# toufique-morshed/CPU-GPU-TFHE

Measured on AMD Instinct MI355X. Metric: gate bootstraps/sec (bootsNAND, N=1024), higher is better.
Workload: dtype f64 (FFT external product; Torus32 in/out, rounded products exact)

## Files before the change

cpu-gpu-tfhe_amd/csrc/keyswitch.hip:

```cpp
#include "engine.h"
#include "modarith.h"

#include <algorithm>
#include <cstdlib>

namespace tfhe_amd {

namespace {


constexpr int kKs4Cols = 4;
constexpr int kKs4Blocks = 126;
constexpr int kKs4I = 32;
#ifndef TFHE_AMD_KS4_THREADS
#define TFHE_AMD_KS4_THREADS 256
#endif
constexpr int kKs4Threads = TFHE_AMD_KS4_THREADS;
constexpr int kKs4ChunkU4 = kKs4I * kKsT * 3;
static_assert(kKs4ChunkU4 % kKs4Threads == 0, "chunk must split evenly");
constexpr int kKs4Pieces = kKs4ChunkU4 / kKs4Threads;

struct KsLane {
    const int32_t *ua, *ua2;
    uint32_t b;
    int32_t *ra, *rb;
};
struct KsPlain {
    const int32_t *u_a, *u_b, *u2_a, *u2_b;
    int32_t add_b;
    int32_t *res_a, *res_b;
    int B;
    __device__ int count() const { return B; }
    __device__ KsLane lane(int ct) const {
        KsLane l;
        l.ua = u_a + (size_t)ct * kN;
        l.ua2 = u2_a ? u2_a + (size_t)ct * kN : nullptr;
        l.b = (uint32_t)u_b[ct] + (uint32_t)add_b + (u2_b ? (uint32_t)u2_b[ct] : 0u);
        l.ra = res_a + (size_t)ct * kn;
        l.rb = res_b + ct;
        return l;
    }
};
struct KsRows {
    const CircKs *ks;
    const int32_t *u_a, *u_b;
    int32_t *wa, *wb;
    int B, nks;
    __device__ int count() const { return B * nks; }
    __device__ KsLane lane(int ct) const {
        const int g = ct / B, k = ct - g * B;
        const CircKs e = ks[g];
        const size_t s1 = (size_t)e.r1 * B + k, so = (size_t)e.out * B + k;
        KsLane l;
        l.ua = u_a + s1 * kN;
        l.b = (uint32_t)u_b[s1] + (uint32_t)e.add_b;
        l.ua2 = nullptr;
        if (e.r2 >= 0) {
            const size_t s2 = (size_t)e.r2 * B + k;
            l.ua2 = u_a + s2 * kN;
            l.b += (uint32_t)u_b[s2];
        }
        l.ra = wa + so * kn;
        l.rb = wb + so;
        return l;
    }
};

template <class P, int SPLIT>
__global__ __launch_bounds__(kKs4Threads) void k_keyswitch_v4(const uint4 *__restrict__ ksk4, P io) {
    __shared__ __attribute__((aligned(16))) uint4 buf[2][kKs4I * kKsT * 4];
    const int part = SPLIT > 1 ? (int)(blockIdx.x % SPLIT) : 0;
    const int bid = SPLIT > 1 ? (int)(blockIdx.x / SPLIT) : (int)blockIdx.x;
    const int xcd = bid & 7, k = bid >> 3;
    const int cb = (k & 15) * 8 + xcd;
    const int ctg = k >> 4;
    if (cb >= kKs4Blocks) return;
    const int tid = threadIdx.x;
    const int ct = ctg * kKs4Threads + tid;
    const bool valid = ct < io.count();
    const KsLane ln = io.lane(valid ? ct : 0);
    for (int t = tid; t < 2 * kKs4I * kKsT; t += kKs4Threads) buf[t >> 8][(t & 255) * 4] = make_uint4(0, 0, 0, 0);

    uint32_t acc[kKs4Cols];
#pragma unroll
    for (int c = 0; c < kKs4Cols; ++c) acc[c] = 0;
    if (SPLIT == 1 && cb * kKs4Cols <= kn && kn < cb * kKs4Cols + kKs4Cols) acc[kn - cb * kKs4Cols] = ln.b;
    constexpr int kIPart = kN / SPLIT;
    const int ibeg = part * kIPart;

    const uint4 *src = ksk4 + ((size_t)cb * kN + ibeg) * kKsT * 3 + tid;
    const uint4 *pa = reinterpret_cast<const uint4 *>(ln.ua + ibeg);
    const uint4 *pa2 = ln.ua2 ? reinterpret_cast<const uint4 *>(ln.ua2 + ibeg) : nullptr;
    int dst[kKs4Pieces];
    uint4 p[kKs4Pieces];
#pragma unroll
    for (int l = 0; l < kKs4Pieces; ++l) {
        const int t = tid + kKs4Threads * l;
        dst[l] = (t / 3) * 4 + (t - 3 * (t / 3)) + 1;
    }
#pragma unroll
    for (int l = 0; l < kKs4Pieces; ++l) p[l] = src[kKs4Threads * l];
    uint4 av[kKs4I / 4], av2[kKs4I / 4];
#pragma unroll
    for (int v = 0; v < kKs4I / 4; ++v) {
        av[v] = pa[v];
        av2[v] = pa2 ? pa2[v] : make_uint4(0, 0, 0, 0);
    }
#pragma unroll
    for (int l = 0; l < kKs4Pieces; ++l) buf[0][dst[l]] = p[l];
    __syncthreads();
    for (int i0 = 0, b = 0; i0 < kIPart; i0 += kKs4I, b ^= 1) {
        uint32_t a[kKs4I];
#pragma unroll
        for (int v = 0; v < kKs4I / 4; ++v) {
            a[4 * v] = av[v].x + av2[v].x + kKsPrecOffset;
            a[4 * v + 1] = av[v].y + av2[v].y + kKsPrecOffset;
            a[4 * v + 2] = av[v].z + av2[v].z + kKsPrecOffset;
            a[4 * v + 3] = av[v].w + av2[v].w + kKsPrecOffset;
        }
        const bool more = i0 + kKs4I < kIPart;
        if (more) {
            const uint4 *sn = src + (size_t)(i0 + kKs4I) * kKsT * 3;
#pragma unroll
            for (int l = 0; l < kKs4Pieces; ++l) p[l] = sn[kKs4Threads * l];
#pragma unroll
            for (int v = 0; v < kKs4I / 4; ++v) {
                av[v] = pa[(i0 + kKs4I) / 4 + v];
                if (pa2) av2[v] = pa2[(i0 + kKs4I) / 4 + v];
            }
        }
        const uint4 *cur = buf[b];
#pragma unroll
        for (int ii = 0; ii < kKs4I; ++ii) {
            const uint32_t ab = a[ii];
#pragma unroll
            for (int j = 0; j < kKsT; ++j) {
                const uint32_t aij = (ab >> (32 - (j + 1) * kKsBasebit)) & (kKsBase - 1);
                const uint4 r = cur[(ii * kKsT + j) * 4 + (int)aij];
                acc[0] -= r.x; acc[1] -= r.y; acc[2] -= r.z; acc[3] -= r.w;
            }
            asm volatile("" : "+v"(acc[0]), "+v"(acc[1]), "+v"(acc[2]), "+v"(acc[3]));
        }
        if (more) {
            uint4 *nb = buf[b ^ 1];
#pragma unroll
            for (int l = 0; l < kKs4Pieces; ++l) nb[dst[l]] = p[l];
        }
        __syncthreads();
    }
    if (!valid) return;
#pragma unroll
    for (int c = 0; c < kKs4Cols; ++c) {
        const int col = cb * kKs4Cols + c;
        int32_t *dst = col < kn ? ln.ra + col : col == kn ? ln.rb : nullptr;
        if (!dst) continue;
        if (SPLIT > 1) atomicAdd(reinterpret_cast<unsigned int *>(dst), acc[c]);
        else *dst = (int32_t)acc[c];
    }
}

constexpr int kKsSmallChunks = 64;
constexpr int kKsSmallI = kN / kKsSmallChunks;

template <class P>
__global__ __launch_bounds__(512) void k_keyswitch_small_init(P io) {
    const KsLane ln = io.lane(blockIdx.x);
    const int col = threadIdx.x;
    if (col < kn) ln.ra[col] = 0;
    else if (col == kn) *ln.rb = (int32_t)ln.b;
}

#ifndef TFHE_AMD_KS_SMALL_U
#define TFHE_AMD_KS_SMALL_U 2
#endif
constexpr int kKsSmallU = TFHE_AMD_KS_SMALL_U;
template <class P, int U>
__global__ __launch_bounds__(512) void k_keyswitch_small(const int32_t *__restrict__ ksk, P io) {
    const int chunk = blockIdx.x, col = threadIdx.x;
    const KsLane ln = io.lane(blockIdx.y);
    if (col > kn) return;
    const int i0 = chunk * kKsSmallI;
    uint32_t acc = 0;
#pragma unroll U
    for (int ii = 0; ii < kKsSmallI; ++ii) {
        const int i = i0 + ii;
        const uint32_t ab = (uint32_t)ln.ua[i] + (ln.ua2 ? (uint32_t)ln.ua2[i] : 0u) + kKsPrecOffset;
        const int32_t *row = ksk + (size_t)i * kKsT * 3 * kKsRow + col;
#pragma unroll
        for (int j = 0; j < kKsT; ++j) {
            const uint32_t h = (ab >> (32 - (j + 1) * kKsBasebit)) & (kKsBase - 1);
            const uint32_t v = (uint32_t)row[(j * 3 + (int)(h ? h : 1u) - 1) * kKsRow];
            acc -= h ? v : 0u;
        }
    }
    int32_t *dst = col < kn ? ln.ra + col : ln.rb;
    atomicAdd(reinterpret_cast<unsigned int *>(dst), acc);
}

typedef int ks5_v4i __attribute__((ext_vector_type(4)));
typedef int ks5_v16i __attribute__((ext_vector_type(16)));
#ifndef TFHE_AMD_KS5_WAVES
#define TFHE_AMD_KS5_WAVES 8
#endif
constexpr int kKs5Waves = TFHE_AMD_KS5_WAVES;
constexpr int kKs5Threads = 64 * kKs5Waves;
constexpr int kKs5Ch = 16;
constexpr int kKs5Nb = 64;
constexpr int kKs5Cols = 8 * kKs5Nb;
static_assert(kKs5Cols > kn, "the N-blocks cover every column and b");
constexpr int kKs5ChU4 = kKs5Ch * 64;
static_assert(kKs5ChU4 % kKs5Threads == 0, "chunk must split evenly");
constexpr int kKs5Pieces = kKs5ChU4 / kKs5Threads;
#ifndef TFHE_AMD_KS5_G
#define TFHE_AMD_KS5_G 8
#endif
constexpr int kKs5G = TFHE_AMD_KS5_G;

template <class P, int SPLIT, int MS>
__global__ __launch_bounds__(kKs5Threads) void k_keyswitch_v5(const uint4 *__restrict__ w5, P io) {
    constexpr int kM = 32 * kKs5Waves * MS;
    constexpr int kG = kKs5G / MS;
    static_assert(kKs5Ch % kG == 0, "groups split the chunk");
    __shared__ __attribute__((aligned(16))) uint2 lut[16][32];
    __shared__ __attribute__((aligned(16))) uint4 bs[2][kKs5Ch][64];
    __shared__ __attribute__((aligned(16))) uint8_t dg[2][2][kM][kKs5Ch];
    const int bid = (int)blockIdx.x, xcd = bid & 7, kk = bid >> 3;
    const int nb = xcd + 8 * (kk & 7), part = (kk >> 3) % SPLIT, mt = (kk >> 3) / SPLIT;
    constexpr int kChunks = kN / kKs5Ch / SPLIT;
    const int c0 = part * kChunks;
    const int tid = threadIdx.x, wave = tid >> 6, l = tid & 63, r = l & 31, hh = l >> 5;
    for (int e = tid; e < 16 * 32; e += kKs5Threads)
        lut[e >> 5][e & 31] = make_uint2(1u << (8 * ((e >> 7) & 3)), 1u << (8 * ((e >> 5) & 3)));
    constexpr int kPer = kKs5Ch * MS / 2;
    constexpr int kU4 = kPer / 4;
    static_assert(kKs5Threads * kPer == kM * kKs5Ch, "loader mapping");
    const int lct = (tid * MS) >> 1, lpart = MS == 1 ? (tid & 1) : 0;
    const int lg = mt * kM + lct;
    const KsLane lln = io.lane(lg < io.count() ? lg : 0);
    const uint4 *pa = reinterpret_cast<const uint4 *>(lln.ua) + kU4 * lpart;
    const uint4 *pa2 = reinterpret_cast<const uint4 *>(lln.ua2 ? lln.ua2 : lln.ua) + kU4 * lpart;
    const uint32_t m2 = lln.ua2 ? 0xffffffffu : 0u;
    pa += c0 * (kKs5Ch / 4);
    pa2 += c0 * (kKs5Ch / 4);
    uint4 uu[kU4], vv[kU4];
#pragma unroll
    for (int q = 0; q < kU4; ++q) {
        uu[q] = pa[q];
        vv[q] = pa2[q];
    }
    auto put_digits = [&](int buf) {
        uint32_t hi[kPer / 4], lo[kPer / 4];
#pragma unroll
        for (int q = 0; q < kU4; ++q) {
            const uint32_t w[4] = {uu[q].x + (vv[q].x & m2) + kKsPrecOffset, uu[q].y + (vv[q].y & m2) + kKsPrecOffset,
                                   uu[q].z + (vv[q].z & m2) + kKsPrecOffset, uu[q].w + (vv[q].w & m2) + kKsPrecOffset};
            hi[q] = (w[0] >> 24) | ((w[1] >> 24) << 8) | ((w[2] >> 24) << 16) | ((w[3] >> 24) << 24);
            lo[q] = ((w[0] >> 16) & 255u) | (((w[1] >> 16) & 255u) << 8) | (((w[2] >> 16) & 255u) << 16) |
                    (((w[3] >> 16) & 255u) << 24);
        }
        if (kU4 == 2) {
            *reinterpret_cast<uint2 *>(&dg[buf][0][lct][kPer * lpart]) = make_uint2(hi[0], hi[1]);
            *reinterpret_cast<uint2 *>(&dg[buf][1][lct][kPer * lpart]) = make_uint2(lo[0], lo[1]);
        } else {
            *reinterpret_cast<uint4 *>(&dg[buf][0][lct][0]) = make_uint4(hi[0], hi[1], hi[2 % kU4], hi[3 % kU4]);
            *reinterpret_cast<uint4 *>(&dg[buf][1][lct][0]) = make_uint4(lo[0], lo[1], lo[2 % kU4], lo[3 % kU4]);
        }
    };
    const uint4 *src = w5 + ((size_t)nb * kN + (size_t)c0 * kKs5Ch) * 64 + tid;
    uint4 p[kKs5Pieces];
#pragma unroll
    for (int q = 0; q < kKs5Pieces; ++q) p[q] = src[q * kKs5Threads];
#pragma unroll
    for (int q = 0; q < kKs5Pieces; ++q) (&bs[0][0][0])[tid + q * kKs5Threads] = p[q];
    put_digits(0);
    __syncthreads();
    ks5_v16i acc[MS];
#pragma unroll
    for (int m = 0; m < MS; ++m) acc[m] = ks5_v16i{};
    for (int c = 0; c < kChunks; ++c) {
        const bool more = c + 1 < kChunks;
        {
            const int cn = more ? c + 1 : c;
            const uint4 *sn = src + (size_t)cn * kKs5ChU4;
#pragma unroll
            for (int q = 0; q < kKs5Pieces; ++q) p[q] = sn[q * kKs5Threads];
#pragma unroll
            for (int q = 0; q < kU4; ++q) {
                uu[q] = pa[cn * (kKs5Ch / 4) + q];
                vv[q] = pa2[cn * (kKs5Ch / 4) + q];
            }
        }
        uint32_t xw[MS][4];
#pragma unroll
        for (int m = 0; m < MS; ++m) {
            const uint4 xd = *reinterpret_cast<const uint4 *>(&dg[c & 1][hh][wave * 32 * MS + 32 * m + r][0]);
            xw[m][0] = xd.x; xw[m][1] = xd.y; xw[m][2] = xd.z; xw[m][3] = xd.w;
        }
        const uint4(*cur)[64] = bs[c & 1];
#pragma unroll
        for (int g = 0; g < kKs5Ch; g += kG) {
            uint4 av[MS][kG], bv[kG];
#pragma unroll
            for (int q = 0; q < kG; ++q) {
                const int ii = g + q;
#pragma unroll
                for (int m = 0; m < MS; ++m) {
                    const uint32_t xb = xw[m][ii >> 2] >> (8 * (ii & 3));
                    const uint2 d01 = lut[(xb >> 4) & 15u][r], d23 = lut[xb & 15u][r];
                    av[m][q] = make_uint4(d01.x, d01.y, d23.x, d23.y);
                }
                bv[q] = cur[ii][l];
            }
            __builtin_amdgcn_sched_barrier(0);
#pragma unroll
            for (int q = 0; q < kG; ++q) {
                const ks5_v4i b = {(int)bv[q].x, (int)bv[q].y, (int)bv[q].z, (int)bv[q].w};
#pragma unroll
                for (int m = 0; m < MS; ++m) {
                    const ks5_v4i a = {(int)av[m][q].x, (int)av[m][q].y, (int)av[m][q].z, (int)av[m][q].w};
                    acc[m] = __builtin_amdgcn_mfma_i32_32x32x32_i8(a, b, acc[m], 0, 0, 0);
                }
            }
        }
        if (more) {
#pragma unroll
            for (int q = 0; q < kKs5Pieces; ++q) (&bs[(c + 1) & 1][0][0])[tid + q * kKs5Threads] = p[q];
            put_digits((c + 1) & 1);
        }
        __syncthreads();
    }
    const int col = nb * 8 + (r >> 2);
    const uint32_t lsh = 8u * (uint32_t)(l & 3);
#pragma unroll
    for (int m = 0; m < MS; ++m) {
#pragma unroll
        for (int reg = 0; reg < 16; ++reg) {
            uint32_t v = (uint32_t)acc[m][reg] << lsh;
            v += (uint32_t)__shfl_xor((int)v, 1, 64);
            v += (uint32_t)__shfl_xor((int)v, 2, 64);
            const int ctm = mt * kM + wave * 32 * MS + 32 * m + (reg & 3) + 8 * (reg >> 2) + 4 * hh;
            if ((l & 3) == 0 && ctm < io.count() && col <= kn) {
                const KsLane lm = io.lane(ctm);
                if (SPLIT > 1) atomicAdd(reinterpret_cast<unsigned int *>(col < kn ? lm.ra + col : lm.rb), 0u - v);
                else if (col < kn) lm.ra[col] = (int32_t)(0u - v);
                else *lm.rb = (int32_t)(lm.b - v);
            }
        }
    }
}

__global__ __launch_bounds__(256) void k_ksk_to_v5(const int32_t *__restrict__ ksk, uint4 *__restrict__ w5) {
    const size_t total = (size_t)kKs5Nb * kN * 64;
    for (size_t t = (size_t)blockIdx.x * 256 + threadIdx.x; t < total; t += (size_t)gridDim.x * 256) {
        const int l = (int)(t & 63);
        const int i = (int)((t >> 6) % kN);
        const int nb = (int)(t / ((size_t)kN * 64));
        const int col = nb * 8 + ((l & 31) >> 2), limb = l & 3, h = l >> 5;
        uint32_t w[4];
#pragma unroll
        for (int tt = 0; tt < 4; ++tt) {
            uint32_t word = 0;
            for (int hh = 1; hh < 4; ++hh) {
                if (col > kn) break;
                uint32_t v = (uint32_t)ksk[(((size_t)i * kKsT + 4 * h + tt) * 3 + (hh - 1)) * kKsRow + col];
                int8_t sb = 0;
                for (int b = 0; b <= limb; ++b) {
                    sb = (int8_t)(v & 0xffu);
                    v = (v - (uint32_t)(int32_t)sb) >> 8;
                }
                word |= (uint32_t)(uint8_t)sb << (8 * hh);
            }
            w[tt] = word;
        }
        w5[t] = make_uint4(w[0], w[1], w[2], w[3]);
    }
}

__global__ __launch_bounds__(256) void k_ksk_to_v4(const int32_t *__restrict__ ksk, uint4 *__restrict__ ksk4) {
    const size_t pieces = (size_t)kKs4Blocks * kN * kKsT * 3;
    for (size_t t = (size_t)blockIdx.x * 256 + threadIdx.x; t < pieces; t += (size_t)gridDim.x * 256) {
        const int cb = (int)(t / ((size_t)kN * kKsT * 3));
        const size_t row = t % ((size_t)kN * kKsT * 3);
        ksk4[t] = *reinterpret_cast<const uint4 *>(ksk + row * kKsRow + cb * kKs4Cols);
    }
}

}

static int ks_split_max() { return 768; }
bool ks5_enabled() {
    static const bool v = [] {
        const char *e = getenv("TFHE_AMD_KS5");
        return !(e && atoi(e) == 0);
    }();
    return v;
}
static int ks5_split(int mtiles) {
    int sp = 1;
    while (sp < 8 && mtiles * kKs5Nb * sp < 512) sp *= 2;
    return sp;
}
template <class P, int MS>
static void launch_ks5(const uint4 *w5, int count, const P &io, hipStream_t s) {
    const int mtiles = (count + 32 * kKs5Waves * MS - 1) / (32 * kKs5Waves * MS);
    const int split = ks5_split(mtiles);
    if (split > 1) hipLaunchKernelGGL(k_keyswitch_small_init<P>, dim3(count), dim3(512), 0, s, io);
    const dim3 grid(mtiles * kKs5Nb * split);
    trace_kernel(split == 8 ? "k_keyswitch_v5(int8-mfma+split8)" : split == 4 ? "k_keyswitch_v5(int8-mfma+split4)"
                 : split == 2 ? "k_keyswitch_v5(int8-mfma+split2)" : "k_keyswitch_v5(int8-mfma)");
    switch (split) {
    case 8: hipLaunchKernelGGL((k_keyswitch_v5<P, 8, MS>), grid, dim3(kKs5Threads), 0, s, w5, io); break;
    case 4: hipLaunchKernelGGL((k_keyswitch_v5<P, 4, MS>), grid, dim3(kKs5Threads), 0, s, w5, io); break;
    case 2: hipLaunchKernelGGL((k_keyswitch_v5<P, 2, MS>), grid, dim3(kKs5Threads), 0, s, w5, io); break;
    default: hipLaunchKernelGGL((k_keyswitch_v5<P, 1, MS>), grid, dim3(kKs5Threads), 0, s, w5, io); break;
    }
}
template <class P>
static void launch_ks4(const DeviceKey &key, int groups, int count, const P &io, hipStream_t s) {
    if (key.ksk5) {
        const uint4 *w5 = reinterpret_cast<const uint4 *>(key.ksk5);
        launch_ks5<P, 1>(w5, count, io, s);
        return;
    }
    trace_kernel("k_keyswitch_v4");
    if (count <= ks_split_max()) {
        hipLaunchKernelGGL(k_keyswitch_small_init<P>, dim3(count), dim3(512), 0, s, io);
        hipLaunchKernelGGL((k_keyswitch_v4<P, 2>), dim3(2 * 128 * groups), dim3(kKs4Threads), 0, s,
                           reinterpret_cast<const uint4 *>(key.ksk4), io);
    } else {
        hipLaunchKernelGGL((k_keyswitch_v4<P, 1>), dim3(128 * groups), dim3(kKs4Threads), 0, s,
                           reinterpret_cast<const uint4 *>(key.ksk4), io);
    }
}

static int ks_unroll_max() { return 4; }

static int ks_small_max() { return ks5_enabled() ? 12 : 96; }

hipError_t launch_keyswitch_rows(const DeviceKey &key, int B, int nks, const CircKs *ks, const int32_t *u_a,
                                 const int32_t *u_b, int32_t *wa, int32_t *wb, hipStream_t s) {
    if (B <= 0 || nks <= 0) return hipSuccess;
    KsRows io{ks, u_a, u_b, wa, wb, B, nks};
    if ((long)B * nks <= ks_small_max()) {
        trace_kernel("k_keyswitch_small");
        hipLaunchKernelGGL(k_keyswitch_small_init<KsRows>, dim3(B * nks), dim3(512), 0, s, io);
        if ((long)B * nks <= ks_unroll_max())
            hipLaunchKernelGGL((k_keyswitch_small<KsRows, kKsSmallI>), dim3(kKsSmallChunks, B * nks), dim3(512), 0, s,
                               key.ksk, io);
        else
            hipLaunchKernelGGL((k_keyswitch_small<KsRows, kKsSmallU>), dim3(kKsSmallChunks, B * nks), dim3(512), 0, s,
                               key.ksk, io);
        return hipGetLastError();
    }
    const int groups = (int)(((size_t)B * nks + kKs4Threads - 1) / kKs4Threads);
    launch_ks4(key, groups, B * nks, io, s);
    return hipGetLastError();
}

__global__ __launch_bounds__(256) void k_circuit_linear(int B, int nlin, const CircLin *__restrict__ lin,
                                                        int32_t *__restrict__ wa, int32_t *__restrict__ wb) {
    const size_t total = (size_t)nlin * B * (kn + 1);
    for (size_t t = (size_t)blockIdx.x * 256 + threadIdx.x; t < total; t += (size_t)gridDim.x * 256) {
        const int w = (int)(t % (kn + 1));
        const size_t gk = t / (kn + 1);
        const int g = (int)(gk / B), k = (int)(gk - (size_t)g * B);
        const CircLin e = lin[g];
        const size_t so = (size_t)e.out * B + k, si = (size_t)(e.in < 0 ? 0 : e.in) * B + k;
        if (w < kn) wa[so * kn + w] = e.in < 0 ? 0 : (int32_t)((uint32_t)e.s * (uint32_t)wa[si * kn + w]);
        else wb[so] = (int32_t)((uint32_t)e.c + (e.in < 0 ? 0u : (uint32_t)e.s * (uint32_t)wb[si]));
    }
}

size_t ksk_v4_words() { return (size_t)kKs4Blocks * kN * kKsT * 3 * 4; }
size_t ksk_v5_words() { return (size_t)kKs5Nb * kN * 64 * 4; }

hipError_t launch_ksk_to_v5(const int32_t *d_ksk, int32_t *d_ksk5, hipStream_t s) {
    hipLaunchKernelGGL(k_ksk_to_v5, dim3(4096), dim3(256), 0, s, d_ksk, reinterpret_cast<uint4 *>(d_ksk5));
    return hipGetLastError();
}

__device__ __forceinline__ double ks_var_one(const int32_t *__restrict__ u, const int32_t *__restrict__ u2,
                                             const double *__restrict__ var) {
    static_assert(kKsT * kKsBasebit == 16 && kKsBase == 4, "digit count below assumes 8 base-4 digits");
    if (var[kKsVarUniform] != 0.0) {
        int k = 0;
#pragma unroll 8
        for (int i = 0; i < kN; ++i) {
            const uint32_t x = ((uint32_t)u[i] + (u2 ? (uint32_t)u2[i] : 0u) + kKsPrecOffset) >> 16;
            k += __builtin_popcount((x | (x >> 1)) & 0x5555u);
        }
        return var[kKsVarUniform + 1 + k];
    }
    double v = 0.0;
    constexpr int U = 4;
    for (int i0 = 0; i0 < kN; i0 += U) {
        uint32_t ab[U];
#pragma unroll
        for (int k = 0; k < U; ++k) ab[k] = (uint32_t)u[i0 + k] + (u2 ? (uint32_t)u2[i0 + k] : 0u) + kKsPrecOffset;
        double t[U][kKsT];
#pragma unroll
        for (int k = 0; k < U; ++k)
#pragma unroll
            for (int j = 0; j < kKsT; ++j) {
                const uint32_t aij = (ab[k] >> (32 - (j + 1) * kKsBasebit)) & (uint32_t)(kKsBase - 1);
                t[k][j] = var[((i0 + k) * kKsT + j) * kKsBase + aij];
            }
#pragma unroll
        for (int k = 0; k < U; ++k)
#pragma unroll
            for (int j = 0; j < kKsT; ++j) {
                const uint32_t aij = (ab[k] >> (32 - (j + 1) * kKsBasebit)) & (uint32_t)(kKsBase - 1);
                v = __dadd_rn(v, aij ? t[k][j] : 0.0);
            }
    }
    return v;
}

__global__ __launch_bounds__(64) void k_ks_variance(const int32_t *__restrict__ u_a, int B, int halves,
                                                    const double *__restrict__ var, double *__restrict__ out) {
    const int g = blockIdx.x * blockDim.x + threadIdx.x;
    if (g >= B) return;
    out[g] = ks_var_one(u_a + (size_t)g * kN, halves == 2 ? u_a + ((size_t)B + g) * kN : nullptr, var);
}

__global__ __launch_bounds__(64) void k_ks_variance_rows(const int32_t *__restrict__ u_a, int B,
                                                         const CircKs *__restrict__ ks, const double *__restrict__ var,
                                                         double *__restrict__ out) {
    const int g = blockIdx.x * blockDim.x + threadIdx.x;
    if (g >= B) return;
    const CircKs k = ks[g];
    out[g] = ks_var_one(u_a + (size_t)k.r1 * kN, k.r2 >= 0 ? u_a + (size_t)k.r2 * kN : nullptr, var);
}

hipError_t launch_ks_variance_rows(const int32_t *u_a, int B, const CircKs *ks, const double *var, double *out,
                                   hipStream_t s) {
    if (B <= 0) return hipSuccess;
    hipLaunchKernelGGL(k_ks_variance_rows, dim3((B + 63) / 64), dim3(64), 0, s, u_a, B, ks, var, out);
    return hipGetLastError();
}

hipError_t launch_ks_variance(const int32_t *u_a, int B, int halves, const double *var, double *out, hipStream_t s) {
    if (B <= 0) return hipSuccess;
    hipLaunchKernelGGL(k_ks_variance, dim3((B + 63) / 64), dim3(64), 0, s, u_a, B, halves, var, out);
    return hipGetLastError();
}

hipError_t launch_circuit_linear(int B, int nlin, const CircLin *lin, int32_t *wa, int32_t *wb, hipStream_t s) {
    if (B <= 0 || nlin <= 0) return hipSuccess;
    const size_t total = (size_t)nlin * B * (kn + 1);
    const int blocks = (int)std::min<size_t>((total + 255) / 256, 65536);
    trace_kernel("k_circuit_linear");
    hipLaunchKernelGGL(k_circuit_linear, dim3(blocks), dim3(256), 0, s, B, nlin, lin, wa, wb);
    return hipGetLastError();
}

hipError_t launch_ksk_to_v4(const int32_t *d_ksk, int32_t *d_ksk4, hipStream_t s) {
    hipLaunchKernelGGL(k_ksk_to_v4, dim3(2048), dim3(256), 0, s, d_ksk, reinterpret_cast<uint4 *>(d_ksk4));
    return hipGetLastError();
}

int ks_version() { return ks5_enabled() ? 5 : 4; }

hipError_t launch_keyswitch(const DeviceKey &key, int B, const int32_t *u_a, const int32_t *u_b,
                            const int32_t *u2_a, const int32_t *u2_b, int32_t add_b,
                            int32_t *res_a, int32_t *res_b, hipStream_t s) {
    if (B <= 0) return hipSuccess;
    if (B <= ks_small_max()) {
        trace_kernel("k_keyswitch_small");
        KsPlain io{u_a, u_b, u2_a, u2_b, add_b, res_a, res_b, B};
        hipLaunchKernelGGL(k_keyswitch_small_init<KsPlain>, dim3(B), dim3(512), 0, s, io);
        if (B <= ks_unroll_max())
            hipLaunchKernelGGL((k_keyswitch_small<KsPlain, kKsSmallI>), dim3(kKsSmallChunks, B), dim3(512), 0, s,
                               key.ksk, io);
        else
            hipLaunchKernelGGL((k_keyswitch_small<KsPlain, kKsSmallU>), dim3(kKsSmallChunks, B), dim3(512), 0, s,
                               key.ksk, io);
    } else {
        const int groups = (B + kKs4Threads - 1) / kKs4Threads;
        KsPlain io{u_a, u_b, u2_a, u2_b, add_b, res_a, res_b, B};
        launch_ks4(key, groups, B, io, s);
    }
    return hipGetLastError();
}

}
```

Baseline: 325,400.

## Stream keyswitch key into LDS ring via async global_load_lds and compute one-hot digits inline

```diff
diff --git a/cpu-gpu-tfhe_amd/csrc/keyswitch.hip b/cpu-gpu-tfhe_amd/csrc/keyswitch.hip
--- a/cpu-gpu-tfhe_amd/csrc/keyswitch.hip
+++ b/cpu-gpu-tfhe_amd/csrc/keyswitch.hip
@@ -199,152 +199,176 @@
 
 typedef int ks5_v4i __attribute__((ext_vector_type(4)));
 typedef int ks5_v16i __attribute__((ext_vector_type(16)));
-#ifndef TFHE_AMD_KS5_WAVES
-#define TFHE_AMD_KS5_WAVES 8
-#endif
-constexpr int kKs5Waves = TFHE_AMD_KS5_WAVES;
+constexpr int kKs5Waves = 8;
 constexpr int kKs5Threads = 64 * kKs5Waves;
-constexpr int kKs5Ch = 16;
+constexpr int kKs5M = 32 * kKs5Waves;
 constexpr int kKs5Nb = 64;
 constexpr int kKs5Cols = 8 * kKs5Nb;
 static_assert(kKs5Cols > kn, "the N-blocks cover every column and b");
-constexpr int kKs5ChU4 = kKs5Ch * 64;
-static_assert(kKs5ChU4 % kKs5Threads == 0, "chunk must split evenly");
-constexpr int kKs5Pieces = kKs5ChU4 / kKs5Threads;
-#ifndef TFHE_AMD_KS5_G
-#define TFHE_AMD_KS5_G 8
+constexpr int kKs5Ring = 3;
+#ifndef TFHE_AMD_KS5_PH
+#define TFHE_AMD_KS5_PH 16
 #endif
-constexpr int kKs5G = TFHE_AMD_KS5_G;
-
-template <class P, int SPLIT, int MS>
+constexpr int kKs5Ph = TFHE_AMD_KS5_PH;
+constexpr int kKs5G = 8;
+
+typedef __attribute__((address_space(3))) void *ks5_lptr;
+
+__device__ __forceinline__ uint32_t ks5_onehot(uint32_t sh, int k, uint32_t one) {
+    uint32_t d;
+    switch (k) {
+    case 0: asm("v_lshlrev_b32_sdwa %0, %1, %2 dst_sel:DWORD dst_unused:UNUSED_PAD src0_sel:BYTE_0 src1_sel:DWORD" : "=v"(d) : "v"(sh), "v"(one)); break;
+    case 1: asm("v_lshlrev_b32_sdwa %0, %1, %2 dst_sel:DWORD dst_unused:UNUSED_PAD src0_sel:BYTE_1 src1_sel:DWORD" : "=v"(d) : "v"(sh), "v"(one)); break;
+    case 2: asm("v_lshlrev_b32_sdwa %0, %1, %2 dst_sel:DWORD dst_unused:UNUSED_PAD src0_sel:BYTE_2 src1_sel:DWORD" : "=v"(d) : "v"(sh), "v"(one)); break;
+    default: asm("v_lshlrev_b32_sdwa %0, %1, %2 dst_sel:DWORD dst_unused:UNUSED_PAD src0_sel:BYTE_3 src1_sel:DWORD" : "=v"(d) : "v"(sh), "v"(one)); break;
+    }
+    return d;
+}
+
+template <class P, int SPLIT, int PH>
 __global__ __launch_bounds__(kKs5Threads) void k_keyswitch_v5(const uint4 *__restrict__ w5, P io) {
-    constexpr int kM = 32 * kKs5Waves * MS;
-    constexpr int kG = kKs5G / MS;
-    static_assert(kKs5Ch % kG == 0, "groups split the chunk");
-    __shared__ __attribute__((aligned(16))) uint2 lut[16][32];
-    __shared__ __attribute__((aligned(16))) uint4 bs[2][kKs5Ch][64];
-    __shared__ __attribute__((aligned(16))) uint8_t dg[2][2][kM][kKs5Ch];
+    constexpr int kM = kKs5M;
+    constexpr int kQ = PH / 16;
+    constexpr int kPhases = kN / PH / SPLIT;
+    static_assert(PH % 16 == 0 && kN % (PH * SPLIT) == 0 && kPhases >= 1, "phases split the range");
+    static_assert(PH % kKs5G == 0 && PH % kKs5Waves == 0, "groups and fill split the phase");
+    constexpr int kOffRing = 0, kOffDg = kKs5Ring * PH * 1024;
+    constexpr int kLds = kOffDg + 2 * 2 * kQ * kM * 16;
+    static_assert(kLds <= 160 * 1024, "LDS of one CU");
+    __shared__ __attribute__((aligned(16))) uint8_t lds[kLds];
+    auto dgp = [&](int buf, int half, int q, int ct) { return lds + kOffDg + (((buf * 2 + half) * kQ + q) * kM + ct) * 16; };
     const int bid = (int)blockIdx.x, xcd = bid & 7, kk = bid >> 3;
     const int nb = xcd + 8 * (kk & 7), part = (kk >> 3) % SPLIT, mt = (kk >> 3) / SPLIT;
-    constexpr int kChunks = kN / kKs5Ch / SPLIT;
-    const int c0 = part * kChunks;
-    const int tid = threadIdx.x, wave = tid >> 6, l = tid & 63, r = l & 31, hh = l >> 5;
-    for (int e = tid; e < 16 * 32; e += kKs5Threads)
-        lut[e >> 5][e & 31] = make_uint2(1u << (8 * ((e >> 7) & 3)), 1u << (8 * ((e >> 5) & 3)));
-    constexpr int kPer = kKs5Ch * MS / 2;
+    const int p0 = part * kPhases;
+    const int tid = threadIdx.x, wave = __builtin_amdgcn_readfirstlane(tid >> 6), l = tid & 63, r = l & 31, hh = l >> 5;
+    const uint4 *src = w5 + ((size_t)nb * kN + (size_t)p0 * PH) * 64 + l;
+    auto fill = [&](int p) {
+        const uint4 *g = src + (size_t)p * PH * 64;
+        const uint32_t slot = __builtin_amdgcn_readfirstlane(
+            (uint32_t)(uintptr_t)(ks5_lptr)(lds + kOffRing + (p % kKs5Ring) * PH * 1024 + wave * 1024));
+#pragma unroll
+        for (int k = 0; k < PH / kKs5Waves; ++k) {
+            uint32_t keep;
+            asm volatile("s_mov_b32 %0, m0\n\ts_mov_b32 m0, %2\n\ts_nop 0\n\tglobal_load_lds_dwordx4 %1, off\n\t"
+                         "s_mov_b32 m0, %0"
+                         : "=&s"(keep)
+                         : "v"(g + (wave + kKs5Waves * k) * 64), "s"(slot + kKs5Waves * k * 1024)
+                         : "memory");
+        }
+    };
+    auto ring_wait = [] { asm volatile("s_waitcnt vmcnt(0)" ::: "memory"); };
+    fill(0);
+    if (kPhases > 1) fill(1);
+    constexpr int kPer = PH / 2;
     constexpr int kU4 = kPer / 4;
-    static_assert(kKs5Threads * kPer == kM * kKs5Ch, "loader mapping");
-    const int lct = (tid * MS) >> 1, lpart = MS == 1 ? (tid & 1) : 0;
+    static_assert(kKs5Threads * kPer == kM * PH, "loader mapping");
+    const int lct = tid >> 1, lpart = tid & 1;
     const int lg = mt * kM + lct;
     const KsLane lln = io.lane(lg < io.count() ? lg : 0);
-    const uint4 *pa = reinterpret_cast<const uint4 *>(lln.ua) + kU4 * lpart;
-    const uint4 *pa2 = reinterpret_cast<const uint4 *>(lln.ua2 ? lln.ua2 : lln.ua) + kU4 * lpart;
-    const uint32_t m2 = lln.ua2 ? 0xffffffffu : 0u;
-    pa += c0 * (kKs5Ch / 4);
-    pa2 += c0 * (kKs5Ch / 4);
+    const uint4 *pa = reinterpret_cast<const uint4 *>(lln.ua) + kU4 * lpart + p0 * (PH / 4);
+    const uint4 *pa2 = reinterpret_cast<const uint4 *>(lln.ua2 ? lln.ua2 : lln.ua) + kU4 * lpart + p0 * (PH / 4);
+    const bool has2 = lln.ua2 != nullptr;
     uint4 uu[kU4], vv[kU4];
 #pragma unroll
     for (int q = 0; q < kU4; ++q) {
         uu[q] = pa[q];
-        vv[q] = pa2[q];
+        vv[q] = make_uint4(0, 0, 0, 0);
+    }
+    if (has2) {
+#pragma unroll
+        for (int q = 0; q < kU4; ++q) vv[q] = pa2[q];
     }
     auto put_digits = [&](int buf) {
-        uint32_t hi[kPer / 4], lo[kPer / 4];
+        uint32_t hi[kU4], lo[kU4];
 #pragma unroll
         for (int q = 0; q < kU4; ++q) {
-            const uint32_t w[4] = {uu[q].x + (vv[q].x & m2) + kKsPrecOffset, uu[q].y + (vv[q].y & m2) + kKsPrecOffset,
-                                   uu[q].z + (vv[q].z & m2) + kKsPrecOffset, uu[q].w + (vv[q].w & m2) + kKsPrecOffset};
+            const uint32_t w[4] = {uu[q].x + vv[q].x + kKsPrecOffset, uu[q].y + vv[q].y + kKsPrecOffset,
+                                   uu[q].z + vv[q].z + kKsPrecOffset, uu[q].w + vv[q].w + kKsPrecOffset};
             hi[q] = (w[0] >> 24) | ((w[1] >> 24) << 8) | ((w[2] >> 24) << 16) | ((w[3] >> 24) << 24);
             lo[q] = ((w[0] >> 16) & 255u) | (((w[1] >> 16) & 255u) << 8) | (((w[2] >> 16) & 255u) << 16) |
                     (((w[3] >> 16) & 255u) << 24);
         }
         if (kU4 == 2) {
-            *reinterpret_cast<uint2 *>(&dg[buf][0][lct][kPer * lpart]) = make_uint2(hi[0], hi[1]);
-            *reinterpret_cast<uint2 *>(&dg[buf][1][lct][kPer * lpart]) = make_uint2(lo[0], lo[1]);
+            *reinterpret_cast<uint2 *>(dgp(buf, 0, 0, lct) + 8 * lpart) = make_uint2(hi[0], hi[1]);
+            *reinterpret_cast<uint2 *>(dgp(buf, 1, 0, lct) + 8 * lpart) = make_uint2(lo[0], lo[1]);
         } else {
-            *reinterpret_cast<uint4 *>(&dg[buf][0][lct][0]) = make_uint4(hi[0], hi[1], hi[2 % kU4], hi[3 % kU4]);
-            *reinterpret_cast<uint4 *>(&dg[buf][1][lct][0]) = make_uint4(lo[0], lo[1], lo[2 % kU4], lo[3 % kU4]);
+            *reinterpret_cast<uint4 *>(dgp(buf, 0, lpart, lct)) = make_uint4(hi[0], hi[1], hi[2 % kU4], hi[3 % kU4]);
+            *reinterpret_cast<uint4 *>(dgp(buf, 1, lpart, lct)) = make_uint4(lo[0], lo[1], lo[2 % kU4], lo[3 % kU4]);
         }
     };
-    const uint4 *src = w5 + ((size_t)nb * kN + (size_t)c0 * kKs5Ch) * 64 + tid;
-    uint4 p[kKs5Pieces];
-#pragma unroll
-    for (int q = 0; q < kKs5Pieces; ++q) p[q] = src[q * kKs5Threads];
-#pragma unroll
-    for (int q = 0; q < kKs5Pieces; ++q) (&bs[0][0][0])[tid + q * kKs5Threads] = p[q];
+    static_assert(kU4 == 2 || kU4 == 4, "PH is 16 or 32");
     put_digits(0);
+    ring_wait();
     __syncthreads();
-    ks5_v16i acc[MS];
-#pragma unroll
-    for (int m = 0; m < MS; ++m) acc[m] = ks5_v16i{};
-    for (int c = 0; c < kChunks; ++c) {
-        const bool more = c + 1 < kChunks;
+    ks5_v16i acc = ks5_v16i{};
+    for (int p = 0; p < kPhases; ++p) {
+        const bool more = p + 1 < kPhases;
+        if (p + 2 < kPhases) fill(p + 2);
         {
-            const int cn = more ? c + 1 : c;
-            const uint4 *sn = src + (size_t)cn * kKs5ChU4;
-#pragma unroll
-            for (int q = 0; q < kKs5Pieces; ++q) p[q] = sn[q * kKs5Threads];
-#pragma unroll
-            for (int q = 0; q < kU4; ++q) {
-                uu[q] = pa[cn * (kKs5Ch / 4) + q];
-                vv[q] = pa2[cn * (kKs5Ch / 4) + q];
-            }
-        }
-        uint32_t xw[MS][4];
-#pragma unroll
-        for (int m = 0; m < MS; ++m) {
-            const uint4 xd = *reinterpret_cast<const uint4 *>(&dg[c & 1][hh][wave * 32 * MS + 32 * m + r][0]);
-            xw[m][0] = xd.x; xw[m][1] = xd.y; xw[m][2] = xd.z; xw[m][3] = xd.w;
-        }
-        const uint4(*cur)[64] = bs[c & 1];
-#pragma unroll
-        for (int g = 0; g < kKs5Ch; g += kG) {
-            uint4 av[MS][kG], bv[kG];
-#pragma unroll
-            for (int q = 0; q < kG; ++q) {
-                const int ii = g + q;
-#pragma unroll
-                for (int m = 0; m < MS; ++m) {
-                    const uint32_t xb = xw[m][ii >> 2] >> (8 * (ii & 3));
-                    const uint2 d01 = lut[(xb >> 4) & 15u][r], d23 = lut[xb & 15u][r];
-                    av[m][q] = make_uint4(d01.x, d01.y, d23.x, d23.y);
+            const int pn = more ? p + 1 : p;
+#pragma unroll
+            for (int q = 0; q < kU4; ++q) uu[q] = pa[pn * (PH / 4) + q];
+            if (has2) {
+#pragma unroll
+                for (int q = 0; q < kU4; ++q) vv[q] = pa2[pn * (PH / 4) + q];
+            }
+        }
+        const uint8_t *cur = lds + kOffRing + (p % kKs5Ring) * PH * 1024 + l * 16;
+#pragma unroll
+        for (int q16 = 0; q16 < kQ; ++q16) {
+            const uint4 xd = *reinterpret_cast<const uint4 *>(dgp(p & 1, hh, q16, wave * 32 + r));
+            const uint32_t xw[4] = {xd.x, xd.y, xd.z, xd.w};
+            uint32_t sh[4][4];
+            const uint32_t one = 1u;
+#pragma unroll
+            for (int d = 0; d < 4; ++d) {
+                const uint32_t m = 0x18181818u;
+                sh[d][0] = (xw[d] >> 3) & m; sh[d][1] = (xw[d] >> 1) & m;
+                sh[d][2] = (xw[d] << 1) & m; sh[d][3] = (xw[d] << 3) & m;
+            }
+#pragma unroll
+            for (int g = 0; g < 16; g += kKs5G) {
+                uint4 av[kKs5G], bv[kKs5G];
+#pragma unroll
+                for (int q = 0; q < kKs5G; ++q) {
+                    const int ii = g + q;
+                    av[q] = make_uint4(ks5_onehot(sh[ii >> 2][0], ii & 3, one), ks5_onehot(sh[ii >> 2][1], ii & 3, one),
+                                       ks5_onehot(sh[ii >> 2][2], ii & 3, one), ks5_onehot(sh[ii >> 2][3], ii & 3, one));
+                    bv[q] = *reinterpret_cast<const uint4 *>(cur + (16 * q16 + ii) * 1024);
                 }
-                bv[q] = cur[ii][l];
-            }
-            __builtin_amdgcn_sched_barrier(0);
-#pragma unroll
-            for (int q = 0; q < kG; ++q) {
-                const ks5_v4i b = {(int)bv[q].x, (int)bv[q].y, (int)bv[q].z, (int)bv[q].w};
-#pragma unroll
-                for (int m = 0; m < MS; ++m) {
-                    const ks5_v4i a = {(int)av[m][q].x, (int)av[m][q].y, (int)av[m][q].z, (int)av[m][q].w};
-                    acc[m] = __builtin_amdgcn_mfma_i32_32x32x32_i8(a, b, acc[m], 0, 0, 0);
+                __builtin_amdgcn_sched_barrier(0);
+#pragma unroll
+                for (int q = 0; q < kKs5G; ++q) {
+                    const ks5_v4i b = {(int)bv[q].x, (int)bv[q].y, (int)bv[q].z, (int)bv[q].w};
+                    const ks5_v4i a = {(int)av[q].x, (int)av[q].y, (int)av[q].z, (int)av[q].w};
+                    acc = __builtin_amdgcn_mfma_i32_32x32x32_i8(a, b, acc, 0, 0, 0);
                 }
             }
         }
+        __builtin_amdgcn_sched_barrier(0);
+#pragma unroll
+        for (int q = 0; q < kU4; ++q)
+            asm volatile("" : "+v"(uu[q].x), "+v"(uu[q].y), "+v"(uu[q].z), "+v"(uu[q].w), "+v"(vv[q].x), "+v"(vv[q].y),
+                              "+v"(vv[q].z), "+v"(vv[q].w));
         if (more) {
-#pragma unroll
-            for (int q = 0; q < kKs5Pieces; ++q) (&bs[(c + 1) & 1][0][0])[tid + q * kKs5Threads] = p[q];
-            put_digits((c + 1) & 1);
-        }
-        __syncthreads();
+            put_digits((p + 1) & 1);
+            ring_wait();
+            __syncthreads();
+        }
     }
     const int col = nb * 8 + (r >> 2);
     const uint32_t lsh = 8u * (uint32_t)(l & 3);
 #pragma unroll
-    for (int m = 0; m < MS; ++m) {
-#pragma unroll
-        for (int reg = 0; reg < 16; ++reg) {
-            uint32_t v = (uint32_t)acc[m][reg] << lsh;
-            v += (uint32_t)__shfl_xor((int)v, 1, 64);
-            v += (uint32_t)__shfl_xor((int)v, 2, 64);
-            const int ctm = mt * kM + wave * 32 * MS + 32 * m + (reg & 3) + 8 * (reg >> 2) + 4 * hh;
-            if ((l & 3) == 0 && ctm < io.count() && col <= kn) {
-                const KsLane lm = io.lane(ctm);
-                if (SPLIT > 1) atomicAdd(reinterpret_cast<unsigned int *>(col < kn ? lm.ra + col : lm.rb), 0u - v);
-                else if (col < kn) lm.ra[col] = (int32_t)(0u - v);
-                else *lm.rb = (int32_t)(lm.b - v);
-            }
+    for (int reg = 0; reg < 16; ++reg) {
+        uint32_t v = (uint32_t)acc[reg] << lsh;
+        v += (uint32_t)__shfl_xor((int)v, 1, 64);
+        v += (uint32_t)__shfl_xor((int)v, 2, 64);
+        const int ctm = mt * kM + wave * 32 + (reg & 3) + 8 * (reg >> 2) + 4 * hh;
+        if ((l & 3) == 0 && ctm < io.count() && col <= kn) {
+            const KsLane lm = io.lane(ctm);
+            if (SPLIT > 1) atomicAdd(reinterpret_cast<unsigned int *>(col < kn ? lm.ra + col : lm.rb), 0u - v);
+            else if (col < kn) lm.ra[col] = (int32_t)(0u - v);
+            else *lm.rb = (int32_t)(lm.b - v);
         }
     }
 }
@@ -396,30 +420,36 @@
     return v;
 }
 static int ks5_split(int mtiles) {
+    static const int forced = [] {
+        const char *e = getenv("TFHE_AMD_KS5_SPLIT");
+        const int v = e ? atoi(e) : 0;
+        return v == 1 || v == 2 || v == 4 || v == 8 ? v : 0;
+    }();
+    if (forced) return forced;
     int sp = 1;
     while (sp < 8 && mtiles * kKs5Nb * sp < 512) sp *= 2;
     return sp;
 }
-template <class P, int MS>
+template <class P>
 static void launch_ks5(const uint4 *w5, int count, const P &io, hipStream_t s) {
-    const int mtiles = (count + 32 * kKs5Waves * MS - 1) / (32 * kKs5Waves * MS);
+    const int mtiles = (count + kKs5M - 1) / kKs5M;
     const int split = ks5_split(mtiles);
     if (split > 1) hipLaunchKernelGGL(k_keyswitch_small_init<P>, dim3(count), dim3(512), 0, s, io);
     const dim3 grid(mtiles * kKs5Nb * split);
     trace_kernel(split == 8 ? "k_keyswitch_v5(int8-mfma+split8)" : split == 4 ? "k_keyswitch_v5(int8-mfma+split4)"
                  : split == 2 ? "k_keyswitch_v5(int8-mfma+split2)" : "k_keyswitch_v5(int8-mfma)");
     switch (split) {
-    case 8: hipLaunchKernelGGL((k_keyswitch_v5<P, 8, MS>), grid, dim3(kKs5Threads), 0, s, w5, io); break;
-    case 4: hipLaunchKernelGGL((k_keyswitch_v5<P, 4, MS>), grid, dim3(kKs5Threads), 0, s, w5, io); break;
-    case 2: hipLaunchKernelGGL((k_keyswitch_v5<P, 2, MS>), grid, dim3(kKs5Threads), 0, s, w5, io); break;
-    default: hipLaunchKernelGGL((k_keyswitch_v5<P, 1, MS>), grid, dim3(kKs5Threads), 0, s, w5, io); break;
+    case 8: hipLaunchKernelGGL((k_keyswitch_v5<P, 8, kKs5Ph>), grid, dim3(kKs5Threads), 0, s, w5, io); break;
+    case 4: hipLaunchKernelGGL((k_keyswitch_v5<P, 4, kKs5Ph>), grid, dim3(kKs5Threads), 0, s, w5, io); break;
+    case 2: hipLaunchKernelGGL((k_keyswitch_v5<P, 2, kKs5Ph>), grid, dim3(kKs5Threads), 0, s, w5, io); break;
+    default: hipLaunchKernelGGL((k_keyswitch_v5<P, 1, kKs5Ph>), grid, dim3(kKs5Threads), 0, s, w5, io); break;
     }
 }
 template <class P>
 static void launch_ks4(const DeviceKey &key, int groups, int count, const P &io, hipStream_t s) {
     if (key.ksk5) {
         const uint4 *w5 = reinterpret_cast<const uint4 *>(key.ksk5);
-        launch_ks5<P, 1>(w5, count, io, s);
+        launch_ks5<P>(w5, count, io, s);
         return;
     }
     trace_kernel("k_keyswitch_v4");
```

Result: no change. 326,300 (median of 2 runs) (+0.3%).
